# kanchan-rihan/llm-sharding-demo

Hardware: AMD Instinct MI355X
Metric: output tokens/sec + p50 per-token latency, GPT-2 pipeline at N MI355X (higher is better)
Workload: dtype bf16; 1 GPU; model=gpt2-xl, global_batch=512, seq_len=256, prompt_len=128, microbatches=2, prefill_chunk=0, parallelism=pp1, sampler=T0.6/top-k40, hipgraphs=True

## Files before the change

csrc/bindings.cpp:

```cpp
#include <torch/extension.h>
#include <c10/hip/HIPStream.h>

#include <hip/hip_runtime.h>
#include <cmath>

#include "kernels/gemm_params.h"

typedef lsd_bf16_t bf16;
using lsd::GemmParams;
using lsd::GemvParams;

extern "C" {
hipError_t lsd_gemm(const GemmParams* p, int epi, int tiled, int* cnt, float* ws, hipStream_t st);
void lsd_gemm_set_big_min(int v);
void lsd_gemm_set_big_group(int v);
void lsd_gemm_set_big_kind(int v);
void lsd_gemm_set_tiled3_max(int v);
void lsd_gemm_set_ring_slots(int v);
void lsd_gemm_set_ring_tn(int v);
void lsd_gemm_set_ring_fill(int v);
void lsd_gemm_set_ring_m96(int v);
void lsd_gemm_set_d256_slots(int v);
void lsd_gemm_set_ring8(int v);
void lsd_gemm_set_ring8_flags(int v);
// ... 25 lines not shown
                            const int* tiles, int n_tiles, const int* seq_slots,
                            const int* q_start, const int* cu_q, bf16* out, long ldo, int nh,
                            int n_kv, int hd, int max_seq, float scale_log2, hipStream_t st);
hipError_t lsd_attn_oproj(const bf16* q, long ldq, const bf16* kc, const bf16* vc,
                          const int* seq_slots, const int* qpos, int B, int nh, int n_kv, int hd,
                          int max_seq, float scale_log2, const bf16* W, long ldw, const bf16* bias,
                          float* x, int N, int NC, float* part, int* cnt, hipStream_t st);
int lsd_gemv_ok(int M, int K, int epi, int norm);
void lsd_gemv_set_nt(int v);
hipError_t lsd_gemv(const lsd::GemvParams* p, int epi, int norm, hipStream_t st);
hipError_t lsd_apply_rows(const int64_t* args, int nargs, int b, hipStream_t st);
hipError_t lsd_silu_mul(const lsd_bf16_t* y, long ldy, lsd_bf16_t* out, long ldo, int M, int F, hipStream_t st);
hipError_t lsd_qkv_post(const float* y, long ldy, const lsd_bf16_t* bias, const int* tslot, const int* tpos,
                        const float* rope, lsd_bf16_t* q, lsd_bf16_t* kc, lsd_bf16_t* vc, int M, int q_size,
                        int kv_size, int hd, int n_kv, int max_seq, hipStream_t st);
hipError_t lsd_sample(const float* logits, long ld, int B, int V, const float* temp,
                      const int* topk, const int* greedy, const long long* seeds,
                      long long* step, int* out, int advance, const int* active, int* pos,
                      const float* segmax, long ldseg, const float* top_p, const float* min_p,
                      hipStream_t st);
}

namespace {

enum Epi : int { EPI_BF16 = 0, EPI_GELU = 1, EPI_SILU_MUL = 2, EPI_F32 = 3, EPI_RESID = 4,
                 EPI_SLAB = 5, EPI_QKV = 6 };

hipStream_t cur_stream() { return c10::hip::getCurrentHIPStream().stream(); }

void check_hip(hipError_t e, const char* what) {
  TORCH_CHECK(e == hipSuccess, what, ": ", hipGetErrorString(e));
}

void need(const torch::Tensor& t, c10::ScalarType dt, const char* name) {
  TORCH_CHECK(t.is_cuda(), name, " must be a GPU tensor");
  TORCH_CHECK(t.scalar_type() == dt, name, " has dtype ", t.scalar_type(), ", expected ", dt);
}

long long* g_stamps = nullptr;

void set_stamps(c10::optional<torch::Tensor> t) {
  if (!t.has_value()) { g_stamps = nullptr; return; }
  need(*t, torch::kInt64, "stamps");
  g_stamps = reinterpret_cast<long long*>(t->data_ptr<int64_t>());
}

void need_rows(const torch::Tensor& t, const char* name) {
  TORCH_CHECK(t.dim() == 2 && t.stride(1) == 1, name, " must be 2-D with unit last stride");
  TORCH_CHECK(t.stride(0) % 8 == 0, name, " row stride must be a multiple of 8 elements");
  TORCH_CHECK(reinterpret_cast<uintptr_t>(t.data_ptr()) % 16 == 0, name, " must be 16-byte aligned");
}

const bf16* bptr(const torch::Tensor& t) { return reinterpret_cast<const bf16*>(t.data_ptr()); }
bf16* bptr_mut(const torch::Tensor& t) { return reinterpret_cast<bf16*>(t.data_ptr()); }

const bf16* opt_bias(const c10::optional<torch::Tensor>& b, int N) {
  if (!b.has_value()) return nullptr;
  need(*b, torch::kBFloat16, "bias");
  TORCH_CHECK(b->is_contiguous() && b->numel() == N, "bias must be contiguous [N]");
  TORCH_CHECK(reinterpret_cast<uintptr_t>(b->data_ptr()) % 16 == 0, "bias must be 16-byte aligned");
  return bptr(*b);
}

int g_slab_bf16 = -1;
bool slab_bf16_enabled() {
  if (g_slab_bf16 < 0) {
    const char* e = std::getenv("LSD_SLAB_BF16");
    g_slab_bf16 = (e == nullptr || e[0] != '0') ? 1 : 0;
  }
  return g_slab_bf16 != 0;
}

GemmParams base_params(const torch::Tensor& a, const torch::Tensor& w, int64_t tiled) {
  need(a, torch::kBFloat16, "a");
  need(w, torch::kBFloat16, "w");
  need_rows(a, "a");
  need_rows(w, "w");
  TORCH_CHECK(a.size(1) == w.size(1), "K mismatch: a ", a.sizes(), " w ", w.sizes());
  GemmParams p{};
  p.A = bptr(a); p.lda = a.stride(0);
  p.W = bptr(w); p.ldw = w.stride(0);
  p.M = a.size(0); p.N = w.size(0); p.K = a.size(1);
  p.splits = 1;
  TORCH_CHECK(p.N % 16 == 0, "N must be a multiple of 16 (pad the weight), got ", p.N);
  TORCH_CHECK(tiled >= 0 && tiled <= 3, "GEMM kind must be 0 (split-K), 1 (tiled), 2 / 3 (256-row), got ", tiled);
  if (tiled >= 2)
    TORCH_CHECK(p.M >= 1 && p.M <= 1024, "256-row-block decode GEMM needs 1 <= M <= 1024, got ", p.M);
  if (tiled) {
    TORCH_CHECK(p.K % 64 == 0, "tiled GEMM needs K % 64 == 0, got ", p.K);
  } else {
    TORCH_CHECK(p.M >= 1 && p.M <= 256, "decode GEMM needs 1 <= M <= 256, got ", p.M);
    TORCH_CHECK(p.K % 32 == 0, "decode GEMM needs K % 32 == 0, got ", p.K);
    TORCH_CHECK(p.N % 64 == 0, "decode GEMM needs N % 64 == 0 (pad the weight), got ", p.N);
  }
  return p;
}

void run_gemm(GemmParams& p, int epi, int64_t tiled, int64_t splits,
              const c10::optional<torch::Tensor>& counters, const torch::Tensor& like,
              const char* what) {
  const int kt = tiled ? p.K / 64 : p.K / 32;
  TORCH_CHECK(splits >= 1 && splits <= kt, what, ": splits must be in [1, ", kt, "], got ", splits);
  p.splits = (int)splits;
  int* cnt = nullptr;
  float* ws = nullptr;
  torch::Tensor wsbuf;
  if (tiled && splits > 1 && epi != EPI_SLAB) {
    const int bn = lsd_gemm_d256_bn((int)tiled, p.M, p.N, p.K);
    const int r8 = tiled == 1 ? lsd_gemm_ring8_tiles(p.M, p.N, p.K, (int)splits) : 0;
    TORCH_CHECK(bn > 0 || r8 > 0, what, ": tiled split-K with an in-kernel combine needs the 256-row "
                "kernel (kind 2 / 3) or the 8-wave decode ring");
    const long tiles = r8 > 0 ? r8 : (long)((p.N + bn - 1) / bn) * ((p.M + 255) / 256);
    const long tile_floats = r8 > 0 ? 128L * 64 : 256L * bn;
    TORCH_CHECK(counters.has_value(), what, ": split-K needs the ticket counter buffer");
    need(*counters, torch::kInt32, "counters");
    TORCH_CHECK(counters->is_contiguous() && counters->numel() >= tiles,
                what, ": counter buffer too small (", counters->numel(), " < ", tiles, ")");
    cnt = counters->data_ptr<int>();
    TORCH_CHECK(splits * tile_floats * 4 < (1L << 31), what, ": split workspace too large");
    wsbuf = torch::empty({tiles * splits * tile_floats}, like.options().dtype(torch::kFloat32));
    ws = wsbuf.data_ptr<float>();
  }
  if (!tiled && epi != EPI_SLAB) {
    const int nw = lsd_gemm_sk_nw(p.M, epi);
    if (epi == EPI_SILU_MUL)
      TORCH_CHECK(p.N % (64 * nw) == 0, what, ": N must be a multiple of ", 64 * nw);
    const long tiles = (p.N + 64 * nw - 1) / (64 * nw) * lsd_gemm_sk_rblocks(p.M, p.N, (int)splits);
    if (splits > 1) {
      TORCH_CHECK(counters.has_value(), what, ": split-K needs the ticket counter buffer");
      need(*counters, torch::kInt32, "counters");
      TORCH_CHECK(counters->is_contiguous() && counters->numel() >= tiles,
                  what, ": counter buffer too small (", counters->numel(), " < ", tiles, ")");
      cnt = counters->data_ptr<int>();
      const long rows = lsd_gemm_sk_rows(p.M, p.N, (int)splits);
      const long bytes = tiles * splits * rows * 64 * nw * 4;
      TORCH_CHECK(splits * rows * 64 * nw * 4 < (1L << 31), what, ": split workspace too large");
      wsbuf = torch::empty({bytes / 4}, like.options().dtype(torch::kFloat32));
      ws = wsbuf.data_ptr<float>();
    }
  }
  p.stamps = g_stamps;
  check_hip(lsd_gemm(&p, epi, (int)tiled, cnt, ws, cur_stream()), what);
}


torch::Tensor linear(torch::Tensor a, torch::Tensor w, c10::optional<torch::Tensor> bias,
                     int64_t act, int64_t tiled, int64_t splits,
                     c10::optional<torch::Tensor> counters) {
  GemmParams p = base_params(a, w, tiled);
  p.bias = opt_bias(bias, p.N);
  int epi = act == 1 ? EPI_GELU : (act == 2 ? EPI_SILU_MUL : EPI_BF16);
  if (epi == EPI_SILU_MUL) TORCH_CHECK(p.N % 32 == 0, "silu_mul needs N % 32 == 0");
  const int n_out = epi == EPI_SILU_MUL ? p.N / 2 : p.N;
  auto out = torch::empty({p.M, n_out}, a.options());
  if (p.M == 0) return out;
  p.out = out.data_ptr(); p.ldo = n_out;
  run_gemm(p, epi, tiled, splits, counters, a, "linear");
  return out;
}

torch::Tensor linear_f32(torch::Tensor a, torch::Tensor w, int64_t tiled, int64_t splits,
                         c10::optional<torch::Tensor> counters, c10::optional<torch::Tensor> segmax) {
  GemmParams p = base_params(a, w, tiled);
  auto out = torch::empty({p.M, p.N}, a.options().dtype(torch::kFloat32));
  if (segmax.has_value()) {
    TORCH_CHECK(tiled != 0, "linear_f32: segment maxima need a tiled kernel");
    need(*segmax, torch::kFloat32, "segmax");
// ... 584 lines not shown
```

csrc/kernels/gemm.hip:

```cpp
#include "common.h"
#include "gemm_params.h"

namespace lsd {

enum Epi : int {
  EPI_BF16 = 0,
  EPI_GELU = 1,
  EPI_SILU_MUL = 2,
  EPI_F32 = 3,
  EPI_RESID = 4,
  EPI_SLAB = 5,
  EPI_QKV = 6,
};


__device__ __forceinline__ void hd_split(int hd, int c, int& head, int& d) {
  if ((hd & (hd - 1)) == 0) {
    head = c >> __builtin_ctz(hd);
    d = c & (hd - 1);
  } else {
    head = c / hd;
    d = c % hd;
  }
}
// ... 101 lines not shown
    const f32x4* x = reinterpret_cast<const f32x4*>(reinterpret_cast<const float*>(p.out) + (long)m * p.ldo + n);
    e.x0 = x[0];
    e.x1 = x[1];
  }
  if constexpr (EPI == EPI_QKV) {
    e.pos = p.tpos[m];
    e.slot = n >= p.q_size ? p.tslot[m] : 0;
  }
}

template <int EPI>
__device__ __forceinline__ void epi8_pre2(const GemmParams& p, int n, Epi8Pre& e) {
  if constexpr (EPI == EPI_QKV) {
    if (p.rope != nullptr && n < p.q_size + p.kv_size) {
      int hh, d0;
      hd_split(p.hd, n < p.q_size ? n : n - p.q_size, hh, d0);
      const f32x4* cs = reinterpret_cast<const f32x4*>(p.rope + ((long)e.pos * (p.hd >> 1) + (d0 >> 1)) * 2);
      e.cs0 = cs[0];
      e.cs1 = cs[1];
    }
  }
}

template <int EPI>
__device__ __forceinline__ void epi8_post(const GemmParams& p, int m, int n, const float* v, int split,
                                          const Epi8Pre& e) {
  if constexpr (EPI == EPI_SLAB) {
    if (p.slab_bf16) {
      bf16x8 o;
#pragma unroll
      for (int j = 0; j < 8; ++j) o[j] = f2bf(v[j]);
      st8(reinterpret_cast<bf16*>(p.slab) + (long)split * p.M * p.N + (long)m * p.N + n, o);
      return;
    }
  }
  if constexpr (EPI == EPI_SLAB || EPI == EPI_F32) {
    float* o = EPI == EPI_SLAB ? p.slab + (long)split * p.M * p.N + (long)m * p.N + n
                               : reinterpret_cast<float*>(p.out) + (long)m * p.ldo + n;
    reinterpret_cast<f32x4*>(o)[0] = f32x4{v[0], v[1], v[2], v[3]};
    reinterpret_cast<f32x4*>(o)[1] = f32x4{v[4], v[5], v[6], v[7]};
    if constexpr (EPI == EPI_F32) {
      if (p.segmax) {
        const float m01 = fmaxf(fmaxf(v[0], v[1]), fmaxf(v[2], v[3]));
        const float m23 = fmaxf(fmaxf(v[4], v[5]), fmaxf(v[6], v[7]));
        p.segmax[(long)m * p.ldseg + (n >> 3)] = fmaxf(m01, m23);
      }
    }
    return;
  }
  float y[8];
  if (p.bias) {
#pragma unroll
    for (int j = 0; j < 8; ++j) y[j] = v[j] + bf2f(e.b[j]);
  } else {
#pragma unroll
    for (int j = 0; j < 8; ++j) y[j] = v[j];
  }
  if constexpr (EPI == EPI_RESID) {
    f32x4* x = reinterpret_cast<f32x4*>(reinterpret_cast<float*>(p.out) + (long)m * p.ldo + n);
    f32x4 x0 = e.x0, x1 = e.x1;
#pragma unroll
    for (int j = 0; j < 4; ++j) { x0[j] += y[j]; x1[j] += y[4 + j]; }
    x[0] = x0;
    x[1] = x1;
    return;
  }
  if constexpr (EPI == EPI_BF16 || EPI == EPI_GELU) {
    bf16x8 o;
#pragma unroll
    for (int j = 0; j < 8; ++j) o[j] = f2bf(EPI == EPI_GELU ? gelu_new(y[j]) : y[j]);
    st8(reinterpret_cast<bf16*>(p.out) + (long)m * p.ldo + n, o);
    return;
  }
  if constexpr (EPI == EPI_QKV) {
    const int qk = p.q_size + p.kv_size;
    if (p.rope != nullptr && n < qk) {
#pragma unroll
      for (int h = 0; h < 2; ++h) {
        const f32x4 t = h ? e.cs1 : e.cs0;
#pragma unroll
        for (int q = 0; q < 2; ++q) {
          const float c = t[2 * q], sn = t[2 * q + 1];
          const float a = y[4 * h + 2 * q], b = y[4 * h + 2 * q + 1];
          y[4 * h + 2 * q] = a * c - b * sn;
          y[4 * h + 2 * q + 1] = b * c + a * sn;
        }
      }
    }
    bf16x8 o;
#pragma unroll
    for (int j = 0; j < 8; ++j) o[j] = f2bf(y[j]);
    if (n < p.q_size) {
      st8(reinterpret_cast<bf16*>(p.out) + (long)m * p.ldo + n, o);
    } else {
      const int c = n < qk ? n - p.q_size : n - qk;
      bf16* cache = n < qk ? p.kc : p.vc;
      int head, d;
      hd_split(p.hd, c, head, d);
      st8(cache + (((long)e.slot * p.n_kv + head) * p.max_seq + e.pos) * p.hd + d, o);
    }
  }
}

template <int EPI>
__device__ __forceinline__ void epilogue8(const GemmParams& p, int m, int n, const float* v, int split) {
  Epi8Pre e;
  epi8_pre<EPI>(p, m, n, e);
  epi8_pre2<EPI>(p, n, e);
  epi8_post<EPI>(p, m, n, v, split, e);
}

template <int EPI, int NCH, int NT, class At>
__device__ __forceinline__ void store_pass(const GemmParams& p, int nchunks, int split, At at) {
  Epi8Pre e[NCH];
  int mm[NCH], nn[NCH];
  const float* sp[NCH];
  bool ok[NCH];
#pragma unroll
  for (int i = 0; i < NCH; ++i) {
    const int c = (int)threadIdx.x + i * NT;
    ok[i] = c < nchunks && at(c, mm[i], nn[i], sp[i]);
    if (ok[i]) epi8_pre<EPI>(p, mm[i], nn[i], e[i]);
  }
  __builtin_amdgcn_s_waitcnt(vmcnt_imm(0));
  if constexpr (EPI == EPI_QKV) {
    if (p.rope != nullptr) {
#pragma unroll
      for (int i = 0; i < NCH; ++i)
        if (ok[i]) epi8_pre2<EPI>(p, nn[i], e[i]);
      __builtin_amdgcn_s_waitcnt(vmcnt_imm(0));
    }
  }
#pragma unroll
  for (int i = 0; i < NCH; ++i) {
    if (!ok[i]) continue;
    const f32x4 lo = *reinterpret_cast<const f32x4*>(sp[i]);
    const f32x4 hi = *reinterpret_cast<const f32x4*>(sp[i] + 4);
    const float v[8] = {lo[0], lo[1], lo[2], lo[3], hi[0], hi[1], hi[2], hi[3]};
    epi8_post<EPI>(p, mm[i], nn[i], v, split, e[i]);
  }
}

template <int MT>
constexpr int sk_round_steps() {
#ifdef LSD_SK_ROUND
  return LSD_SK_ROUND;
#else
  return MT > 4 ? 4 : (MT > 2 ? 8 : 16);
#endif
}
constexpr int LGKM0_SK = 0xC07F;

__device__ __forceinline__ void glds16(const void* g, void* lds) {
  __builtin_amdgcn_global_load_lds((__attribute__((address_space(1))) const void*)g,
                                   (__attribute__((address_space(3))) void*)lds, 16, 0, 0);
}

#define LSD_STAMP(k)                                                                       \
  if (p.stamps && threadIdx.x == 0)                                                        \
    p.stamps[(((long)blockIdx.z * gridDim.y + blockIdx.y) * gridDim.x + blockIdx.x) * 8 + (k)] = \
        __builtin_amdgcn_s_memrealtime();

template <int MT, int NW, int EPI>
__global__ __launch_bounds__(256) void gemm_sk_kernel(GemmParams p, int* __restrict__ cnt,
                                                      float* __restrict__ ws) {
  constexpr int ROWS = MT * 16;
  constexpr int CHUNK_BYTES = ROWS * 256;
  constexpr int BNB = 64 * NW;
  constexpr int SK_ROUND_STEPS = sk_round_steps<MT>();
  constexpr int NCHUNK = SK_ROUND_STEPS / 4;
  __shared__ __attribute__((aligned(16))) char smem[2 * NCHUNK * CHUNK_BYTES + 16];
  int* s_flag = reinterpret_cast<int*>(smem + 2 * NCHUNK * CHUNK_BYTES);

  LSD_STAMP(0)
  if (p.stamps && threadIdx.x == 0)
    p.stamps[(((long)blockIdx.z * gridDim.y + blockIdx.y) * gridDim.x + blockIdx.x) * 8 + 7] =
        __builtin_amdgcn_s_getreg((20 << 0) | (0 << 6) | (3 << 11));
  const int lane = lane_id(), w = threadIdx.x >> 6;
  const int r = lane & 15, g = lane >> 4;
  const int split = blockIdx.y, S = p.splits;
  const int rb0 = blockIdx.z * ROWS;
  const int tile = blockIdx.x;
  const int tile_id = blockIdx.z * gridDim.x + tile;
  const int n_w = tile * BNB + w * 16 * NW;
  const int KT = p.K >> 5;
  const int kb = (int)((long)KT * split / S), ke = (int)((long)KT * (split + 1) / S);

  const bf16* wrow[NW];
#pragma unroll
  for (int ns = 0; ns < NW; ++ns) wrow[ns] = p.W + (long)min(n_w + 16 * ns + r, p.N - 1) * p.ldw + g * 8;

  f32x4 acc[MT][NW];
#pragma unroll
  for (int mt = 0; mt < MT; ++mt)
#pragma unroll
    for (int ns = 0; ns < NW; ++ns) acc[mt][ns] = f32x4{0.f, 0.f, 0.f, 0.f};

  constexpr int LOADS = SK_ROUND_STEPS * NW + NCHUNK * MT;
  static_assert(LOADS <= 63, "vmcnt holds at most 63 outstanding loads");
  constexpr int WAIT_PREV = (LOADS & 0xF) | ((LOADS >> 4) << 14) | (0x7 << 4) | (0xF << 8);
  constexpr int WAIT_ALL = (0x7 << 4) | (0xF << 8);
  constexpr int BUF_BYTES = NCHUNK * CHUNK_BYTES;
  const int nrounds = (ke - kb + SK_ROUND_STEPS - 1) / SK_ROUND_STEPS;

  auto issue = [&](int rd, bf16x8 (&wv)[SK_ROUND_STEPS][NW], char* buf) {
    const int k0 = kb + rd * SK_ROUND_STEPS;
    const int nst = min(SK_ROUND_STEPS, ke - k0);
#pragma unroll
    for (int j = 0; j < SK_ROUND_STEPS; ++j)
#pragma unroll
      for (int ns = 0; ns < NW; ++ns) wv[j][ns] = ld8(wrow[ns] + (long)(k0 + min(j, nst - 1)) * 32);
#pragma unroll
    for (int i = 0; i < NCHUNK * MT; ++i) {
      const int inst = w + 4 * i;
      const int c = inst / (MT * 4), q = inst % (MT * 4);
      const int row = q * 4 + (lane >> 4);
      const int lch = (lane & 15) ^ (row & 15);
      const int kk = min((k0 + min(c * 4, nst - 1)) * 32 + lch * 8, p.K - 8);
      glds16(p.A + (long)min(rb0 + row, p.M - 1) * p.lda + kk, buf + c * CHUNK_BYTES + q * 1024);
    }
  };
  auto compute = [&](int rd, bf16x8 (&wv)[SK_ROUND_STEPS][NW], const char* buf) {
// ... 699 lines not shown
      for (int j = 0; j < 4; ++j) acc[i][j] = mfma16(ac[i], wcur[j], acc[i][j]);
    LSD_PRIO(0);
    __builtin_amdgcn_sched_barrier(0);
    __builtin_amdgcn_s_waitcnt(LGKM0);
  };

  bf16x8 a0[8], w0[4], a1[8], w1[4];
  if (ns > 0) {
#pragma unroll
    for (int q = 0; q < GSLOTS - 1; ++q)
      if (q < ns) stage(q);
    if (ns >= 3) asm volatile("s_waitcnt vmcnt(8)" ::: "memory");
    else if (ns == 2) asm volatile("s_waitcnt vmcnt(4)" ::: "memory");
    else asm volatile("s_waitcnt vmcnt(0)" ::: "memory");
    __builtin_amdgcn_s_barrier();
#pragma unroll
    for (int j = 0; j < 4; ++j) w0[j] = frag_w(0, j);
#pragma unroll
    for (int i = 0; i < 8; ++i) a0[i] = frag_a(0, i);
    __builtin_amdgcn_s_waitcnt(LGKM0);
  }
  for (int s = 0; s < ns; s += 2) {
    step_mma(s, a0, w0, a1, w1);
    step_mma(s + 1, a1, w1, a0, w0);
  }

  float* ct = reinterpret_cast<float*>(smem);
#pragma unroll
  for (int h = 0; h < 2; ++h) {
    if (h == 0) asm volatile("s_waitcnt vmcnt(0) lgkmcnt(0)" ::: "memory");
    else asm volatile("s_waitcnt lgkmcnt(0)" ::: "memory");
    __syncthreads();
    if ((wc >> 1) == h) {
#pragma unroll
      for (int i = 0; i < 8; ++i)
#pragma unroll
        for (int j = 0; j < 4; ++j)
#pragma unroll
          for (int q = 0; q < 4; ++q) {
            const int row = wr * 128 + i * 16 + 4 * g + q;
            const int col = (wc & 1) * 64 + j * 16 + r;
            ct[row * 128 + (col ^ (((row >> 2) & 3) << 4))] = acc[i][j][q];
          }
    }
    __syncthreads();
    if constexpr (EPI != EPI_SILU_MUL) {
      store_pass<EPI, GBM * 16 / 512, 512>(p, GBM * 16, split, [&](int c, int& m, int& n, const float*& src) {
        const int row = c >> 4, ch = c & 15;
        m = m0 + row;
        n = n0 + h * 128 + ch * 8;
        src = ct + row * 128 + ((ch * 8) ^ (((row >> 2) & 3) << 4));
        return m < p.M && n < p.N;
      });
      continue;
    }
    for (int c = threadIdx.x; c < GBM * 16; c += 512) {
      const int row = c >> 4, ch = c & 15, m = m0 + row, n = n0 + h * 128 + ch * 8;
      if (m >= p.M || n >= p.N) continue;
      const float* src = ct + row * 128 + ((ch * 8) ^ (((row >> 2) & 3) << 4));
      const f32x4 lo = *reinterpret_cast<const f32x4*>(src);
      const f32x4 hi = *reinterpret_cast<const f32x4*>(src + 4);
      float v[8] = {lo[0], lo[1], lo[2], lo[3], hi[0], hi[1], hi[2], hi[3]};
      if constexpr (EPI == EPI_SILU_MUL) {
        if ((ch & 3) >= 2) continue;
        const float* up = ct + row * 128 + (((ch + 2) * 8) ^ (((row >> 2) & 3) << 4));
        const f32x4 ulo = *reinterpret_cast<const f32x4*>(up);
        const f32x4 uhi = *reinterpret_cast<const f32x4*>(up + 4);
        const float u[8] = {ulo[0], ulo[1], ulo[2], ulo[3], uhi[0], uhi[1], uhi[2], uhi[3]};
        bf16x8 o;
#pragma unroll
        for (int e = 0; e < 8; ++e) o[e] = f2bf(silu(v[e]) * u[e]);
        st8(reinterpret_cast<bf16*>(p.out) + (long)m * p.ldo + (n >> 5) * 16 + (n & 15), o);
      } else {
        epilogue8<EPI>(p, m, n, v, split);
      }
    }
  }
}

constexpr int P8_HALF = 128 * 64 * 2;
constexpr int P8_BUF = 4 * P8_HALF;
constexpr int P8_SMEM = 2 * P8_BUF;

template <bool BUF = false>
__device__ __forceinline__ void p8_stage(char* lds, const bf16* src, long ld, int row0, int row_max,
                                         int k0) {
  const int lane = lane_id(), w = threadIdx.x >> 6;
  if constexpr (BUF) {
    const __amdgpu_buffer_rsrc_t rs =
        __builtin_amdgcn_make_buffer_rsrc((void*)(src + (long)row0 * ld + k0), 0, 0x7fffffff, 0x00020000);
#pragma unroll
    for (int q = 0; q < 2; ++q) {
      const int inst = w * 2 + q;
      const int row = inst * 8 + (lane >> 3);
      const int lch = (lane & 7) ^ ((row >> 1) & 7);
      const int off = ((min(row0 + row, row_max) - row0) * (int)ld + lch * 8) * 2;
      __builtin_amdgcn_raw_ptr_buffer_load_lds(rs, (lds_void*)(lds + inst * 1024), 16, off, 0, 0, 0);
    }
    return;
  }
#pragma unroll
  for (int q = 0; q < 2; ++q) {
    const int inst = w * 2 + q;
    const int row = inst * 8 + (lane >> 3);
    const int lch = (lane & 7) ^ ((row >> 1) & 7);
    const bf16* gp = src + (long)min(row0 + row, row_max) * ld + k0 + lch * 8;
    __builtin_amdgcn_global_load_lds((gbl_cvoid*)gp, (lds_void*)(lds + inst * 1024), 16, 0, 0);
  }
}

template <int EPI, int VAR = 0>
__global__ __launch_bounds__(512) void gemm_p8_kernel(GemmParams p, int tiles_m, int tiles_n, int G) {
  __shared__ __attribute__((aligned(16))) char smem[P8_SMEM];
  const int nwg = gridDim.x;
  const int bid = xcd_remap(blockIdx.x, nwg);
  const int per_split = tiles_m * tiles_n;
  const int split = bid / per_split;
  int tm, tn;
  tile_order(bid % per_split, tiles_m, tiles_n, G, tm, tn);
  const int m0 = tm * 256, n0 = tn * 256;
  LSD_STAMP(0)
  const int KT = p.K / 64;
  const int kb = (int)((long)KT * split / p.splits);
  const int T = (int)((long)KT * (split + 1) / p.splits) - kb;

  const int lane = lane_id(), w = threadIdx.x >> 6;
  const int wr = w >> 2, wc = w & 3;
  const int r = lane & 15, g = lane >> 4;

  f32x4 acc[8][4];
#pragma unroll
  for (int i = 0; i < 8; ++i)
#pragma unroll
    for (int j = 0; j < 4; ++j) acc[i][j] = f32x4{0.f, 0.f, 0.f, 0.f};

  auto stage = [&](int t, int h) {
    char* dst = smem + (t & 1) * P8_BUF + h * P8_HALF;
    const int k0 = (kb + t) * 64;
    if (h < 2) p8_stage<(VAR & 4) != 0>(dst, p.A, p.lda, m0 + h * 128, p.M - 1, k0);
    else p8_stage<(VAR & 4) != 0>(dst, p.W, p.ldw, n0 + (h - 2) * 128, p.N - 1, k0);
  };
  bf16x8 af[4][2], b0[2][2], b1[2][2];
  auto read_a = [&](int t, int mh) {
    const char* src = smem + (t & 1) * P8_BUF + mh * P8_HALF;
#pragma unroll
    for (int i = 0; i < 4; ++i)
#pragma unroll
      for (int kk = 0; kk < 2; ++kk) af[i][kk] = lds_frag(src, wr * 64 + i * 16 + r, kk * 4 + g);
  };
  auto read_b = [&](int t, int nh, bf16x8 (&bf)[2][2]) {
    const char* src = smem + (t & 1) * P8_BUF + (2 + nh) * P8_HALF;
#pragma unroll
    for (int j = 0; j < 2; ++j)
#pragma unroll
      for (int kk = 0; kk < 2; ++kk) bf[j][kk] = lds_frag(src, wc * 32 + j * 16 + r, kk * 4 + g);
  };
#ifdef LSD_P8_PROF
  long long pf_t0 = 0, pf_vm = 0, pf_b1 = 0, pf_b2 = 0, pf_c = 0;
#define P8_T() __builtin_amdgcn_s_memtime()
#define P8_ACC(acc, stmt) { pf_c = P8_T(); stmt; acc += P8_T() - pf_c; }
#else
#define P8_ACC(acc, stmt) stmt;
#endif
  auto mma = [&](int mh, int nh, bf16x8 (&bf)[2][2]) {
    P8_ACC(pf_b1, __builtin_amdgcn_s_barrier())
    __builtin_amdgcn_s_waitcnt(LGKM0);
    __builtin_amdgcn_sched_barrier(0);
    __builtin_amdgcn_s_setprio(1);
#pragma unroll
    for (int kk = 0; kk < 2; ++kk)
#pragma unroll
      for (int i = 0; i < 4; ++i)
#pragma unroll
        for (int j = 0; j < 2; ++j)
          acc[mh * 4 + i][nh * 2 + j] = mfma16(af[i][kk], bf[j][kk], acc[mh * 4 + i][nh * 2 + j]);
    __builtin_amdgcn_s_setprio(0);
    __builtin_amdgcn_sched_barrier(0);
    P8_ACC(pf_b2, __builtin_amdgcn_s_barrier())
  };

  if (T > 0) {
    stage(0, 0);
    stage(0, 2);
    stage(0, 3);
    stage(0, 1);
    if (T > 1) {
      stage(1, 0);
      stage(1, 2);
      asm volatile("s_waitcnt vmcnt(4)" ::: "memory");
    } else {
      asm volatile("s_waitcnt vmcnt(0)" ::: "memory");
    }
    __builtin_amdgcn_s_barrier();
    LSD_STAMP(1)
    if (wr == 1) __builtin_amdgcn_s_barrier();

#ifdef LSD_P8_PROF
    pf_t0 = P8_T();
#endif
    for (int t = 0; t < T; ++t) {
      const bool n1 = t + 1 < T, n2 = t + 2 < T;
      read_a(t, 0);
      read_b(t, 0, b0);
      if (n1) stage(t + 1, 3);
      __builtin_amdgcn_sched_barrier(0);
      mma(0, 0, b0);
      read_b(t, 1, b1);
      if (n1) stage(t + 1, 1);
      P8_ACC(pf_vm, if (n1) asm volatile("s_waitcnt vmcnt(8)" ::: "memory");
                    else asm volatile("s_waitcnt vmcnt(0)" ::: "memory"))
      __builtin_amdgcn_sched_barrier(0);
      mma(0, 1, b1);
      read_a(t, 1);
      if (n2) stage(t + 2, 0);
      __builtin_amdgcn_sched_barrier(0);
      mma(1, 1, b1);
      if (n2) stage(t + 2, 2);
      P8_ACC(pf_vm, if (n2) asm volatile("s_waitcnt vmcnt(6)" ::: "memory");
                    else if (n1) asm volatile("s_waitcnt vmcnt(2)" ::: "memory"))
      __builtin_amdgcn_sched_barrier(0);
      mma(1, 0, b0);
    }
    if (wr == 0) __builtin_amdgcn_s_barrier();
#ifdef LSD_P8_PROF
    if (p.stamps && threadIdx.x == 0) {
      long long* ps = p.stamps + (long)blockIdx.x * 8;
      ps[4] = P8_T() - pf_t0;
      ps[5] = pf_vm;
      ps[6] = pf_b1;
      ps[7] = pf_b2;
    }
#endif
  }
#undef P8_ACC
  LSD_STAMP(2)

  float* ct = reinterpret_cast<float*>(smem);
#pragma unroll
  for (int h = 0; h < 2; ++h) {
    if (h == 0) asm volatile("s_waitcnt vmcnt(0) lgkmcnt(0)" ::: "memory");
    else asm volatile("s_waitcnt lgkmcnt(0)" ::: "memory");
    __syncthreads();
#pragma unroll
    for (int mh = 0; mh < 2; ++mh)
#pragma unroll
      for (int i = 0; i < 4; ++i)
#pragma unroll
        for (int j = 0; j < 2; ++j)
#pragma unroll
          for (int q = 0; q < 4; ++q) {
            const int row = mh * 128 + wr * 64 + i * 16 + 4 * g + q;
            const int col = wc * 32 + j * 16 + r;
            ct[row * 128 + (col ^ (((row >> 2) & 3) << 4))] = acc[mh * 4 + i][h * 2 + j][q];
          }
    __syncthreads();
    if constexpr (EPI != EPI_SILU_MUL) {
      store_pass<EPI, 256 * 16 / 512, 512>(p, 256 * 16, split, [&](int c, int& m, int& n, const float*& src) {
        const int row = c >> 4, ch = c & 15;
        m = m0 + row;
        n = n0 + h * 128 + ch * 8;
        src = ct + row * 128 + ((ch * 8) ^ (((row >> 2) & 3) << 4));
        return m < p.M && n < p.N;
      });
      continue;
    }
    for (int c = threadIdx.x; c < 256 * 16; c += 512) {
      const int row = c >> 4, ch = c & 15, m = m0 + row, n = n0 + h * 128 + ch * 8;
      if (m >= p.M || n >= p.N) continue;
      const float* src = ct + row * 128 + ((ch * 8) ^ (((row >> 2) & 3) << 4));
      const f32x4 lo = *reinterpret_cast<const f32x4*>(src);
      const f32x4 hi = *reinterpret_cast<const f32x4*>(src + 4);
      float v[8] = {lo[0], lo[1], lo[2], lo[3], hi[0], hi[1], hi[2], hi[3]};
      if constexpr (EPI == EPI_SILU_MUL) {
        if ((ch & 3) >= 2) continue;
        const float* up = ct + row * 128 + (((ch + 2) * 8) ^ (((row >> 2) & 3) << 4));
        const f32x4 ulo = *reinterpret_cast<const f32x4*>(up);
        const f32x4 uhi = *reinterpret_cast<const f32x4*>(up + 4);
        const float u[8] = {ulo[0], ulo[1], ulo[2], ulo[3], uhi[0], uhi[1], uhi[2], uhi[3]};
        bf16x8 o;
#pragma unroll
        for (int e = 0; e < 8; ++e) o[e] = f2bf(silu(v[e]) * u[e]);
        st8(reinterpret_cast<bf16*>(p.out) + (long)m * p.ldo + (n >> 5) * 16 + (n & 15), o);
      } else {
        epilogue8<EPI>(p, m, n, v, split);
      }
    }
  }
  LSD_STAMP(3)
}


template <int ROWS, bool BL = kStageBL>
__device__ __forceinline__ void stage8(char* lds_tile, const bf16* src, long ld, int row0, int row_max,
                                       int k0) {
  stage_rows<ROWS, 8, 0, BL>(lds_tile, src, ld, row0, row_max, k0, threadIdx.x >> 6);
}

template <int BN, int SLOTS>
constexpr int d256_smem() {
  return SLOTS * (256 + BN) * 128 > 256 * (BN + 4) * 4 ? SLOTS * (256 + BN) * 128 : 256 * (BN + 4) * 4;
}

template <int EPI, int BN, int SLOTS>
__global__ __launch_bounds__(512) void gemm_d256_kernel(GemmParams p, int* __restrict__ cnt,
                                                        float* __restrict__ ws) {
  constexpr int NJ = BN / 16;
  constexpr int A_BYTES = 256 * 64 * 2;
  constexpr int SLOT_BYTES = A_BYTES + BN * 64 * 2;
  constexpr int LPS = 4 + BN / 64;
  constexpr int D = SLOTS - 1;
  constexpr int SMEM = d256_smem<BN, SLOTS>();
  static_assert(SLOTS >= 2 && SLOTS <= 4 && SLOTS * SLOT_BYTES <= 160 * 1024, "LDS ring");
  static_assert((D - 1) * LPS <= 63, "vmcnt range");
  __shared__ __attribute__((aligned(16))) char smem[SMEM];
  int* s_flag = reinterpret_cast<int*>(smem);

  const int S = p.splits;
  const int bid = xcd_remap(blockIdx.x, gridDim.x);
  const int tile = bid / S, split = bid % S;
// ... 64 lines not shown
      if (t == S - 1) __hip_atomic_store(cnt + tile, 0, __ATOMIC_RELAXED, __HIP_MEMORY_SCOPE_AGENT);
    }
    __syncthreads();
    if (*s_flag == 0) return;
    LSD_STAMP(2)
#pragma unroll
    for (int i = 0; i < 2; ++i)
#pragma unroll
      for (int j = 0; j < NJ; ++j) acc[i][j] = f32x4{0.f, 0.f, 0.f, 0.f};
    constexpr int RG = 16 / NJ;
    for (int s0 = 0; s0 < S; s0 += RG) {
      f32x4 v[RG][2][NJ];
#pragma unroll
      for (int u = 0; u < RG; ++u) {
        const int s2 = min(s0 + u, S - 1);
#pragma unroll
        for (int i = 0; i < 2; ++i)
#pragma unroll
          for (int j = 0; j < NJ; ++j)
            v[u][i][j] = __builtin_bit_cast(
                f32x4, __builtin_amdgcn_raw_buffer_load_b128(rs, s2 * PER_BLOCK * 16 + (i * NJ + j) * 8192 + toff,
                                                             0, 16));
      }
#pragma unroll
      for (int u = 0; u < RG; ++u) {
        const float msk = (s0 + u < S) ? 1.f : 0.f;
#pragma unroll
        for (int i = 0; i < 2; ++i)
#pragma unroll
          for (int j = 0; j < NJ; ++j) acc[i][j] += v[u][i][j] * msk;
      }
    }
  }

  constexpr int CLD = BN + 4;
  constexpr int CPR = BN / 8;
  __syncthreads();
  float* ct = reinterpret_cast<float*>(smem);
#pragma unroll
  for (int i = 0; i < 2; ++i)
#pragma unroll
    for (int j = 0; j < NJ; ++j)
#pragma unroll
      for (int q = 0; q < 4; ++q) ct[(w * 32 + i * 16 + 4 * g + q) * CLD + j * 16 + r] = acc[i][j][q];
  __syncthreads();
  if constexpr (EPI != EPI_SILU_MUL) {
    store_pass<EPI, (256 * CPR + 511) / 512, 512>(p, 256 * CPR, split, [&](int c, int& m, int& n, const float*& src) {
      const int row = c / CPR, ch = c % CPR;
      m = m0 + row;
      n = n0 + ch * 8;
      src = ct + row * CLD + ch * 8;
      return m < p.M && n < p.N;
    });
    LSD_STAMP(3)
    return;
  }
  for (int c = threadIdx.x; c < 256 * CPR; c += 512) {
    const int row = c / CPR, ch = c % CPR, m = m0 + row, n = n0 + ch * 8;
    if (m >= p.M || n >= p.N) continue;
    const float* src = ct + row * CLD + ch * 8;
    const f32x4 lo = *reinterpret_cast<const f32x4*>(src);
    const f32x4 hi = *reinterpret_cast<const f32x4*>(src + 4);
    float v[8] = {lo[0], lo[1], lo[2], lo[3], hi[0], hi[1], hi[2], hi[3]};
    if constexpr (EPI == EPI_SILU_MUL) {
      if ((ch & 3) >= 2) continue;
      const float* up = src + 16;
      const f32x4 ulo = *reinterpret_cast<const f32x4*>(up);
      const f32x4 uhi = *reinterpret_cast<const f32x4*>(up + 4);
      const float u[8] = {ulo[0], ulo[1], ulo[2], ulo[3], uhi[0], uhi[1], uhi[2], uhi[3]};
      bf16x8 o;
#pragma unroll
      for (int e = 0; e < 8; ++e) o[e] = f2bf(silu(v[e]) * u[e]);
      st8(reinterpret_cast<bf16*>(p.out) + (long)m * p.ldo + (n >> 5) * 16 + (n & 15), o);
    } else {
      epilogue8<EPI>(p, m, n, v, split);
    }
  }
  LSD_STAMP(3)
}


static int g_big_min_blocks = 160;
static int g_big_group = 4;
static int g_big_kind = 4;
static int g_tiled3_max_blocks = 0;
static int g_ring_slots = 3;
static int g_ring_tn = 128;
static int g_ring_fill = 128;
static int g_ring_m96 = 0;
static int g_ring8 = 0;
static int g_ring8_flags = 0;
static int g_ring8_pack = 0;
static int g_d256_slots = 3;
static int g_sk_rows = 64;
static int g_rb_fill = 192;
static int sk_rblocks(int M, int N, int S) {
  const int need = (M + 127) / 128;
  if (M <= g_sk_rows || (N / 64) * S >= g_rb_fill) return need;
  const int rb = (M + g_sk_rows - 1) / g_sk_rows;
  return rb > need ? rb : need;
}
static int sk_mt(int M, int rb) {
  const int mt = ((M + rb - 1) / rb + 15) / 16;
  return mt == 5 || mt == 7 ? mt + 1 : mt;
}

static int g_nw2_rows = 1 << 30;
static int sk_nw(int M, int epi) { return (epi == EPI_SILU_MUL || M > g_nw2_rows) ? 2 : 1; }

template <int EPI, int NW>
static hipError_t launch_sk_nw(const GemmParams& p, int* cnt, float* ws, hipStream_t st) {
  const int RB = sk_rblocks(p.M, p.N, p.splits);
  const int MT = sk_mt(p.M, RB);
  dim3 grid((p.N + 64 * NW - 1) / (64 * NW), p.splits, RB), block(256);
  switch (MT) {
    case 1: hipLaunchKernelGGL((gemm_sk_kernel<1, NW, EPI>), grid, block, 0, st, p, cnt, ws); break;
    case 2: hipLaunchKernelGGL((gemm_sk_kernel<2, NW, EPI>), grid, block, 0, st, p, cnt, ws); break;
    case 3: hipLaunchKernelGGL((gemm_sk_kernel<3, NW, EPI>), grid, block, 0, st, p, cnt, ws); break;
    case 4: hipLaunchKernelGGL((gemm_sk_kernel<4, NW, EPI>), grid, block, 0, st, p, cnt, ws); break;
    case 6: hipLaunchKernelGGL((gemm_sk_kernel<6, NW, EPI>), grid, block, 0, st, p, cnt, ws); break;
    case 8: hipLaunchKernelGGL((gemm_sk_kernel<8, NW, EPI>), grid, block, 0, st, p, cnt, ws); break;
    default: return hipErrorInvalidValue;
  }
  return hipGetLastError();
}

template <int EPI>
static hipError_t launch_sk(const GemmParams& p, int* cnt, float* ws, hipStream_t st) {
  if constexpr (EPI == EPI_SILU_MUL) {
    return launch_sk_nw<EPI, 2>(p, cnt, ws, st);
  } else {
    return sk_nw(p.M, EPI) == 2 ? launch_sk_nw<EPI, 2>(p, cnt, ws, st) : launch_sk_nw<EPI, 1>(p, cnt, ws, st);
  }
}

static int d256_bn(int kind, int M, int N, int K) {
  if (kind < 2 || M < 1 || M > 1024 || K % 64 != 0) return 0;
  return kind == 3 && N % 128 == 0 ? 128 : 64;
}

template <int EPI, int BN>
static hipError_t launch_d256_bn(const GemmParams& p, int* cnt, float* ws, hipStream_t st) {
  const dim3 grid(((p.N + BN - 1) / BN) * ((p.M + 255) / 256) * p.splits), block(512);
  const int slots = BN == 128 ? min(g_d256_slots, 3) : g_d256_slots;
  switch (slots) {
    case 2: hipLaunchKernelGGL((gemm_d256_kernel<EPI, BN, 2>), grid, block, 0, st, p, cnt, ws); break;
    case 4:
      if constexpr (BN == 64) {
        hipLaunchKernelGGL((gemm_d256_kernel<EPI, BN, 4>), grid, block, 0, st, p, cnt, ws);
        break;
      }
      [[fallthrough]];
    default: hipLaunchKernelGGL((gemm_d256_kernel<EPI, BN, 3>), grid, block, 0, st, p, cnt, ws); break;
  }
  return hipGetLastError();
}

template <int EPI>
static hipError_t launch_d256(const GemmParams& p, int kind, int* cnt, float* ws, hipStream_t st) {
  const int bn = d256_bn(kind, p.M, p.N, p.K);
  if (bn == 0) return hipErrorInvalidValue;
  if (p.splits > 1 && EPI != EPI_SLAB && (cnt == nullptr || ws == nullptr)) return hipErrorInvalidValue;
  return bn == 128 ? launch_d256_bn<EPI, 128>(p, cnt, ws, st) : launch_d256_bn<EPI, 64>(p, cnt, ws, st);
}

template <int EPI>
static hipError_t launch_tiled(const GemmParams& p, int* cnt, float* ws, hipStream_t st) {
  const int bm = (p.M + GBM - 1) / GBM, bn = (p.N + GBN - 1) / GBN;
  if (p.M >= GBM && p.K % 64 == 0 && bm * bn * p.splits >= g_big_min_blocks) {
    if (g_big_kind == 1)
      hipLaunchKernelGGL((gemm_p8_kernel<EPI, 0>), dim3(bm * bn * p.splits), dim3(512), 0, st, p, bm, bn,
                         g_big_group);
    else if (g_big_kind == 4)
      hipLaunchKernelGGL((gemm_p8_kernel<EPI, 4>), dim3(bm * bn * p.splits), dim3(512), 0, st, p, bm, bn,
                         g_big_group);
    else
      hipLaunchKernelGGL((gemm_big_kernel<EPI>), dim3(bm * bn * p.splits), dim3(512), 0, st, p, bm, bn,
                         g_big_group);
    return hipGetLastError();
  }
  const int tm = (p.M + TBM - 1) / TBM;
  if (g_ring_tn == 64 || g_ring_tn == 32 || g_ring_tn == 0) {
    const int tn64 = (p.N + 63) / 64;
    const bool narrow = g_ring_tn == 32 || (g_ring_tn == 0 && tm * tn64 * p.splits < g_ring_fill);
    if (narrow && (p.N % 32) == 0) {
      const int tn = (p.N + 31) / 32;
      if (tm * tn * p.splits <= 2 * g_tiled3_max_blocks) {
        hipLaunchKernelGGL((gemm_ring_kernel<EPI, 3, 32>), dim3(tm * tn * p.splits), dim3(256), 0, st, p, tm, tn);
        return hipGetLastError();
      }
    }
    if (p.splits == 1 && p.M > TBM && g_ring_m96 > 0) {
      const int tm96 = (p.M + 95) / 96;
      if (tm96 * tn64 <= g_ring_m96) {
        hipLaunchKernelGGL((gemm_ring_kernel<EPI, 3, 64, 3>), dim3(tm96 * tn64), dim3(256), 0, st, p, tm96, tn64);
        return hipGetLastError();
      }
    }
    if (tm * tn64 * p.splits <= g_tiled3_max_blocks) {
      const dim3 g8(tm * tn64 * p.splits), b8(512);
      const int rot = (g_ring8_flags & 1) != 0;
      const bool combine = p.splits > 1 && EPI != EPI_SLAB;
      if (combine && (g_ring8 != 2 || cnt == nullptr || ws == nullptr)) return hipErrorInvalidValue;
      if (g_ring8 == 1)
        hipLaunchKernelGGL((gemm_ring8_kernel<EPI, 1, 3>), g8, b8, 0, st, p, tm, tn64, rot, cnt, ws);
      else if (g_ring8 == 2 && g_ring8_pack == 1)
        hipLaunchKernelGGL((gemm_ring8_kernel<EPI, 2, 3, 0, 1>), g8, b8, 0, st, p, tm, tn64, rot, cnt, ws);
      else if (g_ring8 == 2 && g_ring8_pack == 2)
        hipLaunchKernelGGL((gemm_ring8_kernel<EPI, 2, 3, 0, 2>), g8, b8, 0, st, p, tm, tn64, rot, cnt, ws);
      else if (g_ring8 == 2 && g_ring8_pack == 3)
        hipLaunchKernelGGL((gemm_ring8_kernel<EPI, 2, 3, 0, 3>), g8, b8, 0, st, p, tm, tn64, rot, cnt, ws);
      else if (g_ring8 == 2 && (g_ring8_flags & 4))
        hipLaunchKernelGGL((gemm_ring8_kernel<EPI, 2, 3, 0, 0, true>), g8, b8, 0, st, p, tm, tn64, rot, cnt, ws);
      else if (g_ring8 == 2 && (g_ring8_flags & 2))
        hipLaunchKernelGGL((gemm_ring8_kernel<EPI, 2, 3, 1>), g8, b8, 0, st, p, tm, tn64, rot, cnt, ws);
      else if (g_ring8 == 2)
        hipLaunchKernelGGL((gemm_ring8_kernel<EPI, 2, 3>), g8, b8, 0, st, p, tm, tn64, rot, cnt, ws);
      else
        hipLaunchKernelGGL((gemm_ring_kernel<EPI, 3, 64>), dim3(tm * tn64 * p.splits), dim3(256), 0, st, p, tm, tn64);
      return hipGetLastError();
    }
  }
  const int tn = (p.N + TBN - 1) / TBN;
  dim3 grid(tm * tn * p.splits), block(256);
  const int cap128 = g_tiled3_max_blocks / 2;
  if (tm * tn * p.splits <= cap128 && g_ring_slots == 4)
    hipLaunchKernelGGL((gemm_ring_kernel<EPI, 4, 128>), grid, block, 0, st, p, tm, tn);
  else if (tm * tn * p.splits <= cap128)
    hipLaunchKernelGGL((gemm_ring_kernel<EPI, 3, 128>), grid, block, 0, st, p, tm, tn);
  else
    hipLaunchKernelGGL((gemm_tiled_kernel<EPI>), grid, block, 0, st, p, tm, tn);
  return hipGetLastError();
}

}

using namespace lsd;

extern "C" void lsd_gemm_set_big_min(int v) { g_big_min_blocks = v; }
extern "C" void lsd_gemm_set_big_group(int v) { g_big_group = v < 0 ? 0 : v; }
extern "C" void lsd_gemm_set_big_kind(int v) { g_big_kind = (v == 1 || v == 4) ? v : 0; }
extern "C" void lsd_gemm_set_tiled3_max(int v) { g_tiled3_max_blocks = v; }
extern "C" void lsd_gemm_set_ring_slots(int v) { g_ring_slots = v == 4 ? 4 : 3; }
extern "C" void lsd_gemm_set_ring_tn(int v) { g_ring_tn = (v == 64 || v == 32 || v == 0) ? v : 128; }
extern "C" void lsd_gemm_set_ring_fill(int v) { g_ring_fill = v; }
extern "C" void lsd_gemm_set_ring_m96(int v) { g_ring_m96 = v; }
extern "C" void lsd_gemm_set_ring8(int v) { g_ring8 = (v == 1 || v == 2) ? v : 0; }
extern "C" void lsd_gemm_set_ring8_flags(int v) { g_ring8_flags = v & 7; }
extern "C" void lsd_gemm_set_ring8_pack(int v) { g_ring8_pack = v & 3; }
extern "C" void lsd_gemm_set_d256_slots(int v) { g_d256_slots = v < 2 ? 2 : (v > 4 ? 4 : v); }

extern "C" int lsd_gemm_d256_bn(int kind, int M, int N, int K) { return d256_bn(kind, M, N, K); }
extern "C" int lsd_gemm_ring8_tiles(int M, int N, int K, int S) {
  if (g_ring8 != 2) return 0;
  const int bm = (M + GBM - 1) / GBM, bn = (N + GBN - 1) / GBN;
  if (M >= GBM && K % 64 == 0 && bm * bn * S >= g_big_min_blocks) return 0;
  if (!(g_ring_tn == 64 || g_ring_tn == 32 || g_ring_tn == 0)) return 0;
  const int tm = (M + TBM - 1) / TBM, tn64 = (N + 63) / 64;
  const bool narrow = g_ring_tn == 32 || (g_ring_tn == 0 && tm * tn64 * S < g_ring_fill);
  if (narrow && (N % 32) == 0 && tm * ((N + 31) / 32) * S <= 2 * g_tiled3_max_blocks) return 0;
  if (S == 1 && M > TBM && g_ring_m96 > 0 && ((M + 95) / 96) * tn64 <= g_ring_m96) return 0;
  return tm * tn64 * S <= g_tiled3_max_blocks ? tm * tn64 : 0;
}
extern "C" int lsd_gemm_sk_rblocks(int M, int N, int S) { return sk_rblocks(M, N, S); }
extern "C" int lsd_gemm_sk_rows(int M, int N, int S) {
  return sk_mt(M, sk_rblocks(M, N, S)) * 16;
}
extern "C" int lsd_gemm_sk_nw(int M, int epi) { return sk_nw(M, epi); }
extern "C" void lsd_gemm_set_nw2_rows(int v) { g_nw2_rows = v; }
extern "C" void lsd_gemm_set_sk_rows(int v) { g_sk_rows = v < 16 ? 16 : (v > 128 ? 128 : v); }

extern "C" hipError_t lsd_gemm(const GemmParams* p, int epi, int kind, int* cnt, float* ws,
                               hipStream_t st) {
#define LSD_DISPATCH(E)                                                                   \
  case E:                                                                                 \
    return kind >= 2 ? launch_d256<E>(*p, kind, cnt, ws, st)                              \
                     : (kind ? launch_tiled<E>(*p, cnt, ws, st) : launch_sk<E>(*p, cnt, ws, st));
  switch (epi) {
    LSD_DISPATCH(EPI_BF16)
    LSD_DISPATCH(EPI_GELU)
    LSD_DISPATCH(EPI_SILU_MUL)
    LSD_DISPATCH(EPI_F32)
    LSD_DISPATCH(EPI_RESID)
    LSD_DISPATCH(EPI_QKV)
    LSD_DISPATCH(EPI_SLAB)
    default: return hipErrorInvalidValue;
  }
#undef LSD_DISPATCH
}
```

Baseline: 51380 tokens/s.

## Store big-GEMM bf16 epilogues directly from registers via swapped MFMA operands

Adds a direct-store epilogue to the large p8 GEMM kernel for bf16, GELU and QKV outputs. The MFMA operands are swapped and the weight rows are permuted at staging, so each lane holds 8 contiguous output columns and can write them straight from registers instead of staging the accumulator through LDS. This is meant to remove the LDS round trip and its barriers in the epilogue, and the new variant is made the default. It also changes the RoPE math to use fma and relaxes the N-alignment check for tiled GEMMs. The risks are more scattered global stores and register pressure in the epilogue.

Measured after the change: 51590 tokens/s (median of 6 runs). Within noise of the previous version (+0.4%).

```diff
diff --git a/csrc/bindings.cpp b/csrc/bindings.cpp
--- a/csrc/bindings.cpp
+++ b/csrc/bindings.cpp
@@ -131,7 +131,8 @@
   p.W = bptr(w); p.ldw = w.stride(0);
   p.M = a.size(0); p.N = w.size(0); p.K = a.size(1);
   p.splits = 1;
-  TORCH_CHECK(p.N % 16 == 0, "N must be a multiple of 16 (pad the weight), got ", p.N);
+  TORCH_CHECK(p.N % (tiled ? 8 : 16) == 0, "N must be a multiple of ", tiled ? 8 : 16,
+              " (pad the weight), got ", p.N);
   TORCH_CHECK(tiled >= 0 && tiled <= 3, "GEMM kind must be 0 (split-K), 1 (tiled), 2 / 3 (256-row), got ", tiled);
   if (tiled >= 2)
     TORCH_CHECK(p.M >= 1 && p.M <= 1024, "256-row-block decode GEMM needs 1 <= M <= 1024, got ", p.M);
diff --git a/csrc/kernels/gemm.hip b/csrc/kernels/gemm.hip
--- a/csrc/kernels/gemm.hip
+++ b/csrc/kernels/gemm.hip
@@ -207,8 +207,8 @@
         for (int q = 0; q < 2; ++q) {
           const float c = t[2 * q], sn = t[2 * q + 1];
           const float a = y[4 * h + 2 * q], b = y[4 * h + 2 * q + 1];
-          y[4 * h + 2 * q] = a * c - b * sn;
-          y[4 * h + 2 * q + 1] = b * c + a * sn;
+          y[4 * h + 2 * q] = __builtin_fmaf(a, c, -(b * sn));
+          y[4 * h + 2 * q + 1] = __builtin_fmaf(b, c, a * sn);
         }
       }
     }
@@ -263,6 +263,56 @@
     const f32x4 hi = *reinterpret_cast<const f32x4*>(sp[i] + 4);
     const float v[8] = {lo[0], lo[1], lo[2], lo[3], hi[0], hi[1], hi[2], hi[3]};
     epi8_post<EPI>(p, mm[i], nn[i], v, split, e[i]);
+  }
+}
+
+constexpr bool epi_direct(int epi) { return epi == EPI_BF16 || epi == EPI_GELU || epi == EPI_QKV; }
+
+__device__ __forceinline__ int direct_perm(int row) {
+  return (row & ~31) | ((row & 12) << 1) | ((row & 16) >> 2) | (row & 3);
+}
+
+template <int EPI, int NB, int G, class Row, class Acc>
+__device__ __forceinline__ void direct_store(const GemmParams& p, int n, int split, Row row, Acc acc) {
+  static_assert(epi_direct(EPI) && NB % G == 0, "bf16-output epilogues only");
+  const bool n_ok = n < p.N;
+  auto post = [&](int i, int m, const Epi8Pre& e) {
+    const f32x4 lo = acc(i, 0), hi = acc(i, 1);
+    const float v[8] = {lo[0], lo[1], lo[2], lo[3], hi[0], hi[1], hi[2], hi[3]};
+    epi8_post<EPI>(p, m, n, v, split, e);
+  };
+  if constexpr (EPI != EPI_QKV) {
+    Epi8Pre e;
+    if (n_ok) epi8_pre<EPI>(p, 0, n, e);
+    __builtin_amdgcn_s_waitcnt(vmcnt_imm(0));
+#pragma unroll
+    for (int i = 0; i < NB; ++i) {
+      const int m = row(i);
+      if (n_ok && m < p.M) post(i, m, e);
+    }
+  } else {
+#pragma unroll
+    for (int g0 = 0; g0 < NB; g0 += G) {
+      Epi8Pre e[G];
+      int mm[G];
+      bool ok[G];
+#pragma unroll
+      for (int u = 0; u < G; ++u) {
+        mm[u] = row(g0 + u);
+        ok[u] = n_ok && mm[u] < p.M;
+        if (ok[u]) epi8_pre<EPI>(p, mm[u], n, e[u]);
+      }
+      __builtin_amdgcn_s_waitcnt(vmcnt_imm(0));
+      if (p.rope != nullptr) {
+#pragma unroll
+        for (int u = 0; u < G; ++u)
+          if (ok[u]) epi8_pre2<EPI>(p, n, e[u]);
+        __builtin_amdgcn_s_waitcnt(vmcnt_imm(0));
+      }
+#pragma unroll
+      for (int u = 0; u < G; ++u)
+        if (ok[u]) post(g0 + u, mm[u], e[u]);
+    }
   }
 }
 
@@ -1128,7 +1178,7 @@
 constexpr int P8_BUF = 4 * P8_HALF;
 constexpr int P8_SMEM = 2 * P8_BUF;
 
-template <bool BUF = false>
+template <bool BUF = false, bool PERM = false>
 __device__ __forceinline__ void p8_stage(char* lds, const bf16* src, long ld, int row0, int row_max,
                                          int k0) {
   const int lane = lane_id(), w = threadIdx.x >> 6;
@@ -1140,7 +1190,8 @@
       const int inst = w * 2 + q;
       const int row = inst * 8 + (lane >> 3);
       const int lch = (lane & 7) ^ ((row >> 1) & 7);
-      const int off = ((min(row0 + row, row_max) - row0) * (int)ld + lch * 8) * 2;
+      const int srow = PERM ? direct_perm(row) : row;
+      const int off = ((min(row0 + srow, row_max) - row0) * (int)ld + lch * 8) * 2;
       __builtin_amdgcn_raw_ptr_buffer_load_lds(rs, (lds_void*)(lds + inst * 1024), 16, off, 0, 0, 0);
     }
     return;
@@ -1150,13 +1201,15 @@
     const int inst = w * 2 + q;
     const int row = inst * 8 + (lane >> 3);
     const int lch = (lane & 7) ^ ((row >> 1) & 7);
-    const bf16* gp = src + (long)min(row0 + row, row_max) * ld + k0 + lch * 8;
+    const int srow = PERM ? direct_perm(row) : row;
+    const bf16* gp = src + (long)min(row0 + srow, row_max) * ld + k0 + lch * 8;
     __builtin_amdgcn_global_load_lds((gbl_cvoid*)gp, (lds_void*)(lds + inst * 1024), 16, 0, 0);
   }
 }
 
 template <int EPI, int VAR = 0>
 __global__ __launch_bounds__(512) void gemm_p8_kernel(GemmParams p, int tiles_m, int tiles_n, int G) {
+  constexpr bool DIRECT = (VAR & 8) != 0 && epi_direct(EPI);
   __shared__ __attribute__((aligned(16))) char smem[P8_SMEM];
   const int nwg = gridDim.x;
   const int bid = xcd_remap(blockIdx.x, nwg);
@@ -1184,7 +1237,7 @@
     char* dst = smem + (t & 1) * P8_BUF + h * P8_HALF;
     const int k0 = (kb + t) * 64;
     if (h < 2) p8_stage<(VAR & 4) != 0>(dst, p.A, p.lda, m0 + h * 128, p.M - 1, k0);
-    else p8_stage<(VAR & 4) != 0>(dst, p.W, p.ldw, n0 + (h - 2) * 128, p.N - 1, k0);
+    else p8_stage<(VAR & 4) != 0, DIRECT>(dst, p.W, p.ldw, n0 + (h - 2) * 128, p.N - 1, k0);
   };
   bf16x8 af[4][2], b0[2][2], b1[2][2];
   auto read_a = [&](int t, int mh) {
@@ -1219,7 +1272,8 @@
       for (int i = 0; i < 4; ++i)
 #pragma unroll
         for (int j = 0; j < 2; ++j)
-          acc[mh * 4 + i][nh * 2 + j] = mfma16(af[i][kk], bf[j][kk], acc[mh * 4 + i][nh * 2 + j]);
+          acc[mh * 4 + i][nh * 2 + j] = DIRECT ? mfma16(bf[j][kk], af[i][kk], acc[mh * 4 + i][nh * 2 + j])
+                                               : mfma16(af[i][kk], bf[j][kk], acc[mh * 4 + i][nh * 2 + j]);
     __builtin_amdgcn_s_setprio(0);
     __builtin_amdgcn_sched_barrier(0);
     P8_ACC(pf_b2, __builtin_amdgcn_s_barrier())
@@ -1281,6 +1335,17 @@
 #undef P8_ACC
   LSD_STAMP(2)
 
+  if constexpr (DIRECT) {
+#pragma unroll
+    for (int nh = 0; nh < 2; ++nh)
+      direct_store<EPI, 8, 4>(
+          p, n0 + nh * 128 + wc * 32 + 8 * g, split,
+          [&](int i) { return m0 + (i >> 2) * 128 + wr * 64 + (i & 3) * 16 + r; },
+          [&](int i, int j) { return acc[i][nh * 2 + j]; });
+    LSD_STAMP(3)
+    return;
+  }
+
   float* ct = reinterpret_cast<float*>(smem);
 #pragma unroll
   for (int h = 0; h < 2; ++h) {
@@ -1511,7 +1576,7 @@
 
 static int g_big_min_blocks = 160;
 static int g_big_group = 4;
-static int g_big_kind = 4;
+static int g_big_kind = 12;
 static int g_tiled3_max_blocks = 0;
 static int g_ring_slots = 3;
 static int g_ring_tn = 128;
@@ -1603,6 +1668,9 @@
     else if (g_big_kind == 4)
       hipLaunchKernelGGL((gemm_p8_kernel<EPI, 4>), dim3(bm * bn * p.splits), dim3(512), 0, st, p, bm, bn,
                          g_big_group);
+    else if (g_big_kind == 12)
+      hipLaunchKernelGGL((gemm_p8_kernel<EPI, epi_direct(EPI) ? 12 : 4>), dim3(bm * bn * p.splits), dim3(512),
+                         0, st, p, bm, bn, g_big_group);
     else
       hipLaunchKernelGGL((gemm_big_kernel<EPI>), dim3(bm * bn * p.splits), dim3(512), 0, st, p, bm, bn,
                          g_big_group);
@@ -1668,7 +1736,7 @@
 
 extern "C" void lsd_gemm_set_big_min(int v) { g_big_min_blocks = v; }
 extern "C" void lsd_gemm_set_big_group(int v) { g_big_group = v < 0 ? 0 : v; }
-extern "C" void lsd_gemm_set_big_kind(int v) { g_big_kind = (v == 1 || v == 4) ? v : 0; }
+extern "C" void lsd_gemm_set_big_kind(int v) { g_big_kind = (v == 1 || v == 4 || v == 12) ? v : 0; }
 extern "C" void lsd_gemm_set_tiled3_max(int v) { g_tiled3_max_blocks = v; }
 extern "C" void lsd_gemm_set_ring_slots(int v) { g_ring_slots = v == 4 ? 4 : 3; }
 extern "C" void lsd_gemm_set_ring_tn(int v) { g_ring_tn = (v == 64 || v == 32 || v == 0) ? v : 128; }
```
